# gereonsuch/gr-FDC

Measured on AMD Instinct MI355X. Metric: complex Msamples/s in, 64k-FFT/256-ch overlap-save; achieved HBM GB/s vs peak, higher is better.
Workload: dtype f32

## Files before the change

### gr-fdc_amd/csrc/fdc_block256.hip

```cpp
#include "fdc_blockcommon.hpp"
#include "fdc_iq.hpp"

namespace fdc {

extern __shared__ __attribute__((aligned(16))) unsigned char fdc_smem_blk[];

typedef unsigned long long u8v __attribute__((ext_vector_type(8)));

template <int P>
struct BlkGeom {
    static_assert(P == 2 || P == 4 || P == 8, "passes of 32 columns: N = 16384, 32768 or 65536");
    static constexpr int kN1 = 32 * P;
    static constexpr int kN = 256 * kN1;
    static constexpr int kJT = P == 8 ? 4 : 8;
    static constexpr int kJB = P == 8 ? 2 : P == 4 ? 4 : 8;
    static constexpr int kLd = P == 2 ? 32 * P + 2 : 32 * P + 6;
    static constexpr int kTripBytes = 16 * kJT * kLd * 8;
    static constexpr int kOffCt = kTripBytes > kStripsEnd ? kTripBytes : kStripsEnd;
    static constexpr int kOffWrow = P == 8 ? 136960 : kOffCt + 32 * P * 8;
    static constexpr int kOffB = kOffWrow + 16 * 18 * 8;
    static constexpr int kOffSA = kOffB + 32 * 18 * 8;
    static constexpr int kOffSoff = kOffSA + 16 * P * 18 * 8;
    static constexpr int kLds = kOffSoff + kN1 * 4;
    static constexpr int kOffSoffOff = kOffSA + 16 * P * 16 * 8;
    static constexpr int kOffWrowF = kOffSoffOff + kN1 * 4;
    static constexpr int kLdsOff = kOffWrowF + 16 * 18 * 8;
    static_assert(kLdsOff <= 160 * 1024 && kLds <= 160 * 1024, "LDS budget");
    static_assert(kOffCt >= kStripsEnd && kOffCt + 32 * P * 8 <= kOffWrow, "stage-2 trip buffer and twiddles below the tables, tables above the strips");
    static_assert((16 * (kJB - 1) * kLd + 32 * (P - 1)) * 8 < 65536, "ds offsets of a base register");
};


template <int P, bool NT, bool OFF, bool FWD, bool R4 = false, bool HALF = false, class TI = float2, class TO = float2>
__global__ FDC_PLAIN_DS __launch_bounds__(512, (P == 2 && !OFF && !R4 && !FWD) ? 4 : 2) void k_blk256(const TI *__restrict__ in, size_t in_stride, TO *__restrict__ out,
                                                const float2 *__restrict__ tw256, const float2 *__restrict__ twq,
                                                const float2 *__restrict__ cbt, const float *__restrict__ shn,
                                                const long long *__restrict__ slot_off, long long out_base,
                                                long long nb_call, unsigned out_bytes, int nb, int hints,
                                                unsigned long long *__restrict__ dbg , int roff, long long first_block,
                                                float2 *__restrict__ fwd_scratch, const unsigned *__restrict__ keep,
                                                typename IqTail<TI, TO>::type gpow )
{
    typedef BlkGeom<P> GM;
    constexpr bool kIq = !std::is_same<TI, float2>::value, kOq = !std::is_same<TO, float2>::value;
    static_assert(!kIq || !FWD, "integer input: the channelizer forms (the forward transform takes widened input)");
    static_assert(!kOq || !FWD, "integer output: the channelizer forms");
    constexpr unsigned kEs = (unsigned)sizeof(TI);
    constexpr unsigned kOs = (unsigned)sizeof(TO);
    [[maybe_unused]] const float iq_scale = iq_tail_scale(gpow);
    [[maybe_unused]] const float oq_scale = oq_tail_scale(gpow);
    static_assert(!HALF || (!OFF && !FWD), "the half-slot form is a variant of the on-grid channelizer");
    constexpr int kN1 = GM::kN1, kLd = GM::kLd, kJT = GM::kJT, kJB = GM::kJB;
    float2 *scr = reinterpret_cast<float2 *>(fdc_smem_blk);
    float2 *wrow = reinterpret_cast<float2 *>(fdc_smem_blk + GM::kOffWrow);
    float2 *Bt = reinterpret_cast<float2 *>(fdc_smem_blk + GM::kOffB);
    float2 *SA = reinterpret_cast<float2 *>(fdc_smem_blk + GM::kOffSA);
    constexpr int kSaLd = OFF ? 16 : 18;
    unsigned *soff = reinterpret_cast<unsigned *>(fdc_smem_blk + (OFF ? GM::kOffSoffOff : GM::kOffSoff));
    float2 *ctab = reinterpret_cast<float2 *>(fdc_smem_blk + GM::kOffCt);
    const int tid = threadIdx.x;
    const int w = tid >> 6, lane = tid & 63, col = lane & 3, b = lane >> 2, c5 = 4 * w + col;
    unsigned mqs[4] = {~0u, ~0u, ~0u, ~0u};
    if (FWD && keep) {
        const int wu = __builtin_amdgcn_readfirstlane(w) % P;
#pragma unroll
        for (int q = 0; q < 4; q++) mqs[q] = keep[wu * 4 + q];
    }

    const int grid = gridDim.x, first = xcd_first_block();
    if (first >= nb) return;

    constexpr unsigned inbytes = (unsigned)GM::kN * kEs;
    constexpr unsigned kRowGrp = (unsigned)kN1 * 16u * kEs;
    const unsigned voff = (unsigned)(b * kN1 + c5) * kEs;
    [[maybe_unused]] auto ld_in = [&](__amdgpu_buffer_rsrc_t r, unsigned soff, auto aux) __attribute__((always_inline)) -> cf {
        constexpr int kAux = decltype(aux)::value;
        if constexpr (sizeof(TI) == 4) return mk(__uint_as_float(__builtin_amdgcn_raw_buffer_load_b32(r, voff, soff, kAux)), 0.f);
        else return mk(__uint_as_float((unsigned)__builtin_amdgcn_raw_buffer_load_b16(r, voff, soff, kAux)), 0.f);
    };
    const __amdgpu_buffer_rsrc_t rcb = make_rsrc(cbt, (unsigned)kN1 * 16u * 8u);
    const unsigned voffc = (unsigned)(c5 * 16 + b) * 8u;
    cf LA[16], LB[16], cbA, cbB;
    {
        const __amdgpu_buffer_rsrc_t rin = make_rsrc(in + (size_t)first * in_stride, inbytes);
#pragma unroll
        for (int a = 0; a < 16; a++) {
            if constexpr (kIq) LA[a] = ld_in(rin, (unsigned)a * kRowGrp, std::integral_constant<int, 0>{});
            else LA[a] = bld2(rin, voff, (unsigned)a * kRowGrp);
        }
        cbA = bld2(rcb, voffc, 0);
    }
    float2 *wrowF = OFF ? reinterpret_cast<float2 *>(fdc_smem_blk + GM::kOffWrowF) : wrow;
    const int r16 = roff & 15;
    for (int i = tid; i < 256; i += 512) {
        wrow[(i >> 4) * 18 + (i & 15)] = tw256[((i >> 4) * (i & 15)) & 255];
        if (OFF)
            wrowF[(i >> 4) * 18 + (i & 15)] = tw256[((i >> 4) * ((((i & 15) - r16) & 15) + roff)) & 255];
    }
    for (int i = tid; i < kN1; i += 512) {
        const long long o = slot_off[i];
        soff[(i % P) * 32 + ((i / P) & 1) * 16 + rev16((i / P) >> 1)] = o >= 0 ? (unsigned)((o * nb_call + out_base) * kOs) : 0xFFFFFFFFu;
    }
    for (int i = tid; i < 32 * P; i += 512) ctab[i] = tw256[((i / P) * (i % P) * (8 / P)) & 255];
    Bt[(tid >> 4) * 18 + (tid & 15)] = twq[HALF ? tid ^ 8 : tid];
    for (int i = tid; i < 256 * P; i += 512) {
        const int ps = i >> 8, bb = (i >> 4) & 15, q = i & 15, qt = HALF ? q ^ 8 : q;
        const float2 t = twq[(size_t)(32 * ps) * 16 + qt];
        const float s = shn[bb + 16 * qt];
        SA[(ps * 16 + bb) * kSaLd + q] = make_float2(t.x * s, t.y * s);
    }
    __syncthreads();

    float2 *const scrw = scr + w * kStripPts + lane;
    const float2 *const scrr = scr + w * kStripPts + col + 68 * b;
    const float2 *const wr = wrow + b * 18;
    const float2 *const wrf = wrowF + b * 18;
    const float2 *const btr = Bt + c5 * 18;
    const __amdgpu_buffer_rsrc_t rout = make_rsrc(out, out_bytes);
    constexpr bool kScr = FWD || R4;
    const __amdgpu_buffer_rsrc_t rscr = make_rsrc(kScr ? fwd_scratch + (size_t)blockIdx.x * 32768 : fwd_scratch, kScr ? 32768u * 8u : 0u);


    for (int m = first; m < nb; m += grid) {
        const int mnext = m + grid < nb ? m + grid : m;
        const float sgn = (OFF && !R4 && (roff & 1) && ((first_block + m) & 1)) ? -1.0f : 1.0f;
        cf phs = mk(1.f, 0.f);
        if constexpr (OFF && R4) {
            const int pc = (int)((((first_block + m) & 3) * (roff & 3)) & 3);
            phs = mk(pc == 0 ? 1.f : pc == 2 ? -1.f : 0.f, pc == 1 ? 1.f : pc == 3 ? -1.f : 0.f);
        }
        typedef unsigned long long gvec __attribute__((ext_vector_type(P)));
        gvec G[8];
#define FDC_GGET(j, ps) unpack_cf(G[j][ps])
#define FDC_GPUT(j, ps, val) G[j][ps] = pack_cf(val)
        auto one_pass = [&](const int ps, cf (&cur)[16], const cf cbc, cf (&L)[16], cf &cbn) __attribute__((always_inline)) {
            const cf cb = (OFF && R4) ? cmul(cbc, phs) : OFF ? cbc * sgn : cbc;
            const int pn = ps < P - 1 ? ps + 1 : 0;
            const int mb = ps < P - 1 ? m : mnext;
            const __amdgpu_buffer_rsrc_t rin = make_rsrc(in + (size_t)mb * in_stride + 32 * pn, inbytes);
            if constexpr (kIq) {
                if (hints & 2) {
#pragma unroll
                    for (int a = 0; a < 16; a++) L[a] = ld_in(rin, (unsigned)a * kRowGrp, std::integral_constant<int, 2>{});
                } else {
#pragma unroll
                    for (int a = 0; a < 16; a++) L[a] = ld_in(rin, (unsigned)a * kRowGrp, std::integral_constant<int, 0>{});
                }
            } else if (hints & 2) {
#pragma unroll
                for (int a = 0; a < 16; a++) L[a] = bld2_nt(rin, voff, (unsigned)a * kRowGrp);
            } else {
#pragma unroll
                for (int a = 0; a < 16; a++) L[a] = bld2(rin, voff, (unsigned)a * kRowGrp);
            }
            cbn = bld2(rcb, voffc, (unsigned)pn * 4096u);
            if constexpr (kIq) {
#pragma unroll
                for (int a = 0; a < 16; a++) cur[a] = iq_widen_bits(TI{}, __float_as_uint(cur[a].x), iq_scale);
            }
            dft16<false>(cur);
            cf tw[16];
#pragma unroll
            for (int i = 0; i < 8; i++) {
                const float4 t = ld4(&wrf[2 * i]);
                tw[2 * i] = mk(t.x, t.y); tw[2 * i + 1] = mk(t.z, t.w);
            }
            if (OFF) {
#pragma unroll
                for (int p = 0; p < 16; p++) st2(&scrw[68 * ((p - r16) & 15)], cmul(cur[rev16(p)], tw[p]));
            } else {
                st2(&scrw[0], cur[rev16(0)]);
#pragma unroll
                for (int p = 1; p < 16; p++) st2(&scrw[68 * p], cmul(cur[rev16(p)], tw[p]));
            }
            __builtin_amdgcn_wave_barrier();
            cf v[16];
            strip_get(v, scrr);
            if constexpr (FWD) {
                dft16<false>(v);
                const float2 *sar = SA + (ps * 16 + b) * kSaLd;
#pragma unroll
                for (int i = 0; i < 8; i++) {
                    const float4 t0 = ld4(&btr[2 * i]), t1 = ld4(&sar[2 * i]);
                    const cf y0 = cmul(cmul(cmul(v[rev16(2 * i)], mk(t0.x, t0.y)), mk(t1.x, t1.y)), cb);
                    const cf y1 = cmul(cmul(cmul(v[rev16(2 * i + 1)], mk(t0.z, t0.w)), mk(t1.z, t1.w)), cb);
                    if (i < 4) { FDC_GPUT(2 * i, ps, y0); FDC_GPUT(2 * i + 1, ps, y1); }
                    else {
                        bst2(rscr, (unsigned)tid * 8u + (unsigned)(2 * i - 8) * 4096u, (unsigned)ps * 32768u, y0);
                        bst2(rscr, (unsigned)tid * 8u + (unsigned)(2 * i - 7) * 4096u, (unsigned)ps * 32768u, y1);
                    }
                }
            } else {
                dft16<false>(v);
                cf u[16];
                {
                    const float2 *sar = SA + (ps * 16 + b) * kSaLd;
#pragma unroll
                    for (int i = 0; i < 8; i++) {
                        const float4 t0 = ld4(&btr[2 * i]), t1 = ld4(&sar[2 * i]);
                        u[HALF ? 2 * i : (2 * i) ^ 8] = cmul(cmul(v[rev16(2 * i)], mk(t0.x, t0.y)), mk(t1.x, t1.y));
                        u[HALF ? 2 * i + 1 : (2 * i + 1) ^ 8] = cmul(cmul(v[rev16(2 * i + 1)], mk(t0.z, t0.w)), mk(t1.z, t1.w));
                    }
                }
                dft16<true>(u);
#pragma unroll
                for (int i = 0; i < 8; i++) {
                    const float4 t = ld4(&wr[2 * i]);
                    tw[2 * i] = mk(t.x, t.y); tw[2 * i + 1] = mk(t.z, t.w);
                }
                u[rev16(0)] = cmul(u[rev16(0)], cb);
#pragma unroll
                for (int p = 1; p < 16; p++) u[rev16(p)] = cmul(cmulc(u[rev16(p)], tw[p]), cb);
                strip_trip(u, scrw, scrr);
                dft16<true>(u);
#pragma unroll
                for (int j = 0; j < 8; j++) FDC_GPUT(j, ps, u[rev16(8 + j)]);
                if constexpr (R4) {
#pragma unroll
                    for (int j = 0; j < 4; j++) bst2(rscr, (unsigned)tid * 8u + (unsigned)j * 4096u, (unsigned)ps * 16384u, u[rev16(4 + j)]);
                }
            }
        };
        if constexpr (OFF && P == 8) {
#pragma nounroll
            for (int ps = 0; ps < P; ps++) {
                cf cur[16];
#pragma unroll
                for (int a = 0; a < 16; a++) cur[a] = LA[a];
                one_pass(ps, cur, cbA, LA, cbA);
            }
        } else {
#pragma nounroll
            for (int pp = 0; pp < P; pp += 2) {
                one_pass(pp, LA, cbA, LB, cbB);
                one_pass(pp + 1, LB, cbB, LA, cbA);
            }
        }
        auto stage2 = [&](auto get, const int rowbase, auto njc) __attribute__((always_inline)) {
            constexpr int kNJ = decltype(njc)::value;
            constexpr int kNTrip = (kNJ + kJT - 1) / kJT;
            __syncthreads();
            int t2 = tid;
            asm volatile("" : "+v"(t2));
            const int lane2 = t2 & 63, w2 = __builtin_amdgcn_readfirstlane(t2 >> 6), b_2 = lane2 >> 2, c5_2 = 4 * w2 + (lane2 & 3);
            const int klo2 = w2 % P, rh2 = w2 / P;
            float2 *const gw0 = scr + b_2 * kLd + c5_2;
            int rowjb = 16 * kJB * kLd;
            asm volatile("" : "+v"(rowjb));
            float2 *const gw1 = gw0 + rowjb;
            const float2 *const gr = scr + (64 * rh2 + lane2) * kLd + 32 * klo2;
            const uint4 *const sow = reinterpret_cast<const uint4 *>(soff + 32 * klo2);
#pragma unroll
            for (int tr = 0; tr < kNTrip; tr++) {
                const int ja = kNJ - kJT * tr < kJT ? kNJ - kJT * tr : kJT;
                cf ct[P];
                {
                    const float2 *ctr = reinterpret_cast<const float2 *>(fdc_smem_blk + GM::kOffCt) + c5_2 * P;
#pragma unroll
                    for (int i = 0; i < P / 2; i++) {
                        const float4 t = ld4(&ctr[2 * i]);
                        ct[2 * i] = mk(t.x, t.y); ct[2 * i + 1] = mk(t.z, t.w);
                    }
                }
                cf src[kJT][P];
#pragma unroll
                for (int jj = 0; jj < kJT; jj++)
#pragma unroll
                    for (int ps = 0; ps < P; ps++) if (jj < ja) src[jj][ps] = get(kJT * tr + jj, ps);
#pragma unroll
                for (int jj = 0; jj < kJT; jj++) {
                    if (jj >= ja) continue;
                    cf a[P];
#pragma unroll
                    for (int ps = 0; ps < P; ps++) a[ps] = src[jj][ps];
                    pass_dft<P>(a);
                    float2 *const gw = (jj < kJB ? gw0 : gw1) + (jj % kJB) * 16 * kLd;
                    st2(&gw[0], a[0]);
#pragma unroll
                    for (int k = 1; k < P; k++) st2(&gw[32 * k], cmul(a[pass_idx<P>(k)], ct[k]));
                }
                __builtin_amdgcn_sched_barrier(0);
                __syncthreads();
                const bool reads = P == 8 || 4 * rh2 < ja;
                cf v[32];
                if (reads) {
#pragma unroll
                    for (int i = 0; i < 16; i++) {
                        const float4 t = ld4(&gr[2 * i]);
                        v[2 * i] = mk(t.x, t.y); v[2 * i + 1] = mk(t.z, t.w);
                    }
                }
                __syncthreads();
                __builtin_amdgcn_sched_barrier(0);
                if (reads) {
                    dft32<false>(v);
                    const int trow0 = 16 * kJT * tr + 64 * rh2, trow = trow0 + lane2;
                    const unsigned rb = (unsigned)(m * (FWD ? GM::kN : (R4 ? 192 : 128)) + rowbase + trow) * kOs;
                    unsigned mq = FWD ? mqs[((rowbase + trow0) >> 6) & 3] : ~0u;
                    if constexpr (FWD) asm volatile("" : "+s"(mq));
#pragma unroll
                    for (int q = 0; q < 8; q++) {
                        const uint4 t = sow[q];
                        const unsigned so[4] = {t.x, t.y, t.z, t.w};
#pragma unroll
                        for (int e = 0; e < 4; e++) {
                            const unsigned o = FWD ? (so[e] | (((mq >> (4 * q + e)) & 1u) - 1u)) : so[e];
                            if constexpr (kOq) {
                                const unsigned u = oq_bits(TO{}, v[4 * q + e], oq_scale);
                                if constexpr (kOs == 4) __builtin_amdgcn_raw_buffer_store_b32(u, rout, (o == 0xFFFFFFFFu ? 0xFFFFFFF0u : o + rb), 0, NT ? 2 : 0);
                                else __builtin_amdgcn_raw_buffer_store_b16((unsigned short)u, rout, (o == 0xFFFFFFFFu ? 0xFFFFFFF0u : o + rb), 0, NT ? 2 : 0);
                            } else
                                bst2t<NT>(rout, (o == 0xFFFFFFFFu ? 0xFFFFFFF0u : o + rb), v[4 * q + e]);
                        }
                    }
                    if constexpr (FWD) {
                        if (gpow) {
                            float t16[16];
#pragma unroll
                            for (int i = 0; i < 16; i++) {
                                const float s0 = __builtin_fmaf(v[i].y, v[i].y, v[i].x * v[i].x);
                                const float s1 = __builtin_fmaf(v[i + 16].y, v[i + 16].y, v[i + 16].x * v[i + 16].x);
                                asm("s_nop 1\n\tv_add_f32_dpp %0, %1, %1 row_ror:8 row_mask:0xf bank_mask:0x3\n\t"
                                    "v_add_f32_dpp %0, %2, %2 row_ror:8 row_mask:0xf bank_mask:0xc" : "=&v"(t16[i]) : "v"(s0), "v"(s1));
                            }
                            float t8[8];
#pragma unroll
                            for (int i = 0; i < 8; i++)
                                asm("s_nop 1\n\tv_add_f32_dpp %0, %1, %1 row_shl:4 row_mask:0xf bank_mask:0x5\n\t"
                                    "v_add_f32_dpp %0, %2, %2 row_shr:4 row_mask:0xf bank_mask:0xa" : "=&v"(t8[i]) : "v"(t16[i]), "v"(t16[i + 8]));
                            const bool b1 = (lane2 & 2) != 0, b0 = (lane2 & 1) != 0;
                            float t4[4], t2[2];
#pragma unroll
                            for (int i = 0; i < 4; i++) {
                                const float keepv = b1 ? t8[i + 4] : t8[i], send = b1 ? t8[i] : t8[i + 4];
                                t4[i] = keepv + __builtin_bit_cast(float, __builtin_amdgcn_update_dpp(0, __builtin_bit_cast(int, send), 0x4E , 0xF, 0xF, false));
                            }
#pragma unroll
                            for (int i = 0; i < 2; i++) {
                                const float keepv = b0 ? t4[i + 2] : t4[i], send = b0 ? t4[i] : t4[i + 2];
                                t2[i] = keepv + __builtin_bit_cast(float, __builtin_amdgcn_update_dpp(0, __builtin_bit_cast(int, send), 0xB1 , 0xF, 0xF, false));
                            }
                            const int i16 = lane2 & 15, rho = lane2 >> 4, gsrc = 2 * (i16 & 1);
                            const int a0 = (16 * gsrc + 4 * rho + (i16 >> 2)) * 4, a1 = a0 + 64;
                            const int z0 = __builtin_bit_cast(int, t2[0]), z1 = __builtin_bit_cast(int, t2[1]);
                            const int f0a = __builtin_amdgcn_ds_bpermute(a0, z0), f0b = __builtin_amdgcn_ds_bpermute(a0, z1);
                            const int f1a = __builtin_amdgcn_ds_bpermute(a1, z0), f1b = __builtin_amdgcn_ds_bpermute(a1, z1);
                            const bool odd = (i16 & 2) != 0;
                            float2 pr;
                            pr.x = __builtin_bit_cast(float, odd ? f0b : f0a);
                            pr.y = __builtin_bit_cast(float, odd ? f1b : f1a);
                            const int reg = 8 * rho + (i16 >> 1), slot = klo2 + P * ((reg >> 4) + 2 * (4 * (reg & 3) + ((reg & 15) >> 2)));
                            *reinterpret_cast<float2 *>(gpow + (size_t)m * (GM::kN / 16) + 16 * slot + (rowbase + trow0) / 16 + gsrc) = pr;
                        }
                    }
                }
                __builtin_amdgcn_sched_barrier(0);
            }
        };
        stage2([&](int j, int ps) { return FDC_GGET(j, ps); }, R4 ? 64 : 0, std::integral_constant<int, 8>{});
        if constexpr (FWD) {
            asm volatile("s_waitcnt vmcnt(0)" ::: "memory");
            stage2([&](int j, int ps) { return bld2_sc1(rscr, (unsigned)tid * 8u + (unsigned)(j * 4096 + ps * 32768), 0u); }, 128,
                   std::integral_constant<int, 8>{});
        }
        if constexpr (R4) {
            asm volatile("s_waitcnt vmcnt(0)" ::: "memory");
            stage2([&](int j, int ps) { return bld2_sc1(rscr, (unsigned)tid * 8u + (unsigned)(j * 4096 + ps * 16384), 0u); }, 0,
                   std::integral_constant<int, 4>{});
        }
    }
}

template <class TI>
static hipError_t init_block_kernels_in()
{
    hipError_t e;
#define FDC_SETB(P, A, B, R4) \
    e = hipFuncSetAttribute(reinterpret_cast<const void *>(k_blk256<P, A, B, false, R4, false, TI>), hipFuncAttributeMaxDynamicSharedMemorySize, \
                            B ? BlkGeom<P>::kLdsOff : BlkGeom<P>::kLds); \
    if (e != hipSuccess) return e;
#define FDC_SETH(P, A, R4) \
    e = hipFuncSetAttribute(reinterpret_cast<const void *>(k_blk256<P, A, false, false, R4, true, TI>), hipFuncAttributeMaxDynamicSharedMemorySize, BlkGeom<P>::kLds); \
    if (e != hipSuccess) return e;
#define FDC_SETP(P) \
    FDC_SETB(P, true, false, false) FDC_SETB(P, false, false, false) FDC_SETB(P, true, true, false) FDC_SETB(P, false, true, false) \
    FDC_SETB(P, true, false, true) FDC_SETB(P, false, false, true) FDC_SETB(P, true, true, true) FDC_SETB(P, false, true, true) \
    FDC_SETH(P, true, false) FDC_SETH(P, false, false) FDC_SETH(P, true, true) FDC_SETH(P, false, true)
    FDC_SETP(2) FDC_SETP(4) FDC_SETP(8)
#undef FDC_SETP
#undef FDC_SETH
#undef FDC_SETB
    return hipSuccess;
}

template <class TI, class TO> struct kOqR4Narrowed {
    static constexpr bool value = std::is_same<TI, float2>::value && !std::is_same<TO, float2>::value;
};

template <class TI, class TO>
static hipError_t init_block_kernels_oq()
{
    hipError_t e;
#define FDC_SETB(P, B, R4) \
    e = hipFuncSetAttribute(reinterpret_cast<const void *>(k_blk256<P, true, B, false, R4, false, TI, TO>), hipFuncAttributeMaxDynamicSharedMemorySize, \
                            B ? BlkGeom<P>::kLdsOff : BlkGeom<P>::kLds); \
    if (e != hipSuccess) return e;
#define FDC_SETH(P, R4) \
    e = hipFuncSetAttribute(reinterpret_cast<const void *>(k_blk256<P, true, false, false, R4, true, TI, TO>), hipFuncAttributeMaxDynamicSharedMemorySize, BlkGeom<P>::kLds); \
    if (e != hipSuccess) return e;
#define FDC_SETP(P) \
    FDC_SETB(P, false, false) FDC_SETB(P, true, false) FDC_SETB(P, false, true) FDC_SETB(P, true, true) FDC_SETH(P, false) FDC_SETH(P, true)
    FDC_SETP(2) FDC_SETP(4)
    FDC_SETB(8, false, false) FDC_SETB(8, true, false) FDC_SETH(8, false)
    if constexpr (!kOqR4Narrowed<TI, TO>::value) { FDC_SETB(8, false, true) FDC_SETB(8, true, true) FDC_SETH(8, true) }
#undef FDC_SETP
#undef FDC_SETH
#undef FDC_SETB
    return hipSuccess;
}

hipError_t init_block_kernels()
{
    hipError_t e = init_block_kernels_in<sc16>();
    if (e != hipSuccess) return e;
    if ((e = init_block_kernels_in<sc8>()) != hipSuccess) return e;
    if ((e = init_block_kernels_oq<float2, sc16>()) != hipSuccess) return e;
    if ((e = init_block_kernels_oq<float2, sc8>()) != hipSuccess) return e;
    if ((e = init_block_kernels_oq<sc16, sc16>()) != hipSuccess) return e;
    if ((e = init_block_kernels_oq<sc16, sc8>()) != hipSuccess) return e;
    if ((e = init_block_kernels_oq<sc8, sc16>()) != hipSuccess) return e;
    if ((e = init_block_kernels_oq<sc8, sc8>()) != hipSuccess) return e;
#define FDC_SETB(P, A, B, F, R4) \
    e = hipFuncSetAttribute(reinterpret_cast<const void *>(k_blk256<P, A, B, F, R4>), hipFuncAttributeMaxDynamicSharedMemorySize, \
                            B ? BlkGeom<P>::kLdsOff : BlkGeom<P>::kLds); \
    if (e != hipSuccess) return e;
#define FDC_SETP(P) \
    FDC_SETB(P, true, false, false, false) FDC_SETB(P, false, false, false, false) FDC_SETB(P, true, true, false, false) \
    FDC_SETB(P, false, true, false, false) FDC_SETB(P, true, false, false, true) FDC_SETB(P, false, false, false, true) \
    FDC_SETB(P, true, true, false, true) FDC_SETB(P, false, true, false, true)
    FDC_SETP(2) FDC_SETP(4) FDC_SETP(8)
    FDC_SETB(8, true, false, true, false) FDC_SETB(8, false, false, true, false) FDC_SETB(4, true, false, true, false) FDC_SETB(4, false, false, true, false)
    FDC_SETB(2, true, false, true, false) FDC_SETB(2, false, false, true, false)
#undef FDC_SETP
#undef FDC_SETB
#define FDC_SETH(P, A, R4) \
    e = hipFuncSetAttribute(reinterpret_cast<const void *>(k_blk256<P, A, false, false, R4, true>), hipFuncAttributeMaxDynamicSharedMemorySize, BlkGeom<P>::kLds); \
    if (e != hipSuccess) return e;
#define FDC_SETHP(P) FDC_SETH(P, true, false) FDC_SETH(P, false, false) FDC_SETH(P, true, true) FDC_SETH(P, false, true)
    FDC_SETHP(2) FDC_SETHP(4) FDC_SETHP(8)
#undef FDC_SETHP
#undef FDC_SETH
    return hipSuccess;
}

bool poly_block_supports(int N) { return N == 16384 || N == 32768 || N == 65536; }

template <class TI, class TO = float2>
static hipError_t poly_block_in(const BlockLaunch &b, const TI *in, TO *out, float iq_scale, float oq_scale = 1.0f)
{
    if (b.nb_chunk <= 0) return hipSuccess;
    if (b.L != 256 || b.r < 0 || b.r >= 256) return hipErrorInvalidValue;
    constexpr bool kIq = !std::is_same<TI, float2>::value, kOq = !std::is_same<TO, float2>::value;
    const bool nt = (b.hints & 1) != 0, r4 = b.R == 4;
    if (kOq && !nt) return hipErrorInvalidValue;
    auto iq_tail = [](float si, float so) -> typename IqTail<TI, TO>::type {
        if constexpr (!kIq && !kOq) return (void)si, (void)so, (float *)nullptr;
        else if constexpr (kIq && kOq) return make_float2(si, so);
        else if constexpr (kIq) return (void)so, si;
        else return (void)si, so;
    };
    const bool halfslot = b.half();
    if (!poly_block_supports(b.N) || (b.R != 2 && !r4) || (r4 && !b.scratch)) return hipErrorInvalidValue;
    const int grid = b.grid(b.N == 16384 && b.R == 2 && (!b.r || halfslot) ? 2 : 1);
#define FDC_L(P, A, O, R4, H, roff) \
    hipExtLaunchKernelGGL((k_blk256<P, A || kOq, O, false, R4, H, TI, TO>), dim3((unsigned)grid), dim3(512), O ? BlkGeom<P>::kLdsOff : BlkGeom<P>::kLds, b.s, \
                          b.ev_start, b.ev_stop, 0u, in, b.in_stride, out, b.tw256, b.twq, b.cbt, b.shn, b.slot_off, (long long)b.mbase * (R4 ? 192 : 128), \
                          (long long)b.nb_call, b.out_bytes, b.nb_chunk, b.hints, (unsigned long long *)nullptr, roff, b.first_block, \
                          R4 ? b.scratch : (float2 *)nullptr, (const unsigned *)nullptr, iq_tail(iq_scale, oq_scale))
#define FDC_LB(P, A, O, R4) FDC_L(P, A, O, R4, false, b.r)
#define FDC_LH(P, A, R4) FDC_L(P, A, false, R4, true, 0)
#define FDC_R4(P) if constexpr (P != 8 || !kOqR4Narrowed<TI, TO>::value)
#define FDC_LP(P) \
    do { \
        if (halfslot) { \
            if (r4) { FDC_R4(P) { if (nt) FDC_LH(P, true, true); else FDC_LH(P, false, true); } else return hipErrorInvalidValue; } \
            else { if (nt) FDC_LH(P, true, false); else FDC_LH(P, false, false); } \
        } else if (r4 && b.r) { FDC_R4(P) { if (nt) FDC_LB(P, true, true, true); else FDC_LB(P, false, true, true); } else return hipErrorInvalidValue; } \
        else if (r4) { FDC_R4(P) { if (nt) FDC_LB(P, true, false, true); else FDC_LB(P, false, false, true); } else return hipErrorInvalidValue; } \
        else if (b.r) { if (nt) FDC_LB(P, true, true, false); else FDC_LB(P, false, true, false); } \
        else { if (nt) FDC_LB(P, true, false, false); else FDC_LB(P, false, false, false); } \
    } while (0)
    if (b.N == 65536) FDC_LP(8); else if (b.N == 32768) FDC_LP(4); else FDC_LP(2);
#undef FDC_LP
#undef FDC_R4
#undef FDC_LH
#undef FDC_LB
#undef FDC_L
    return hipGetLastError();
}

hipError_t launch_poly_block(const BlockLaunch &b) { return poly_block_in(b, b.in, b.out, 1.0f); }

hipError_t launch_poly_block_iq(const BlockLaunch &b, int fmt, float scale, const void *in)
{
    if (fmt == kIqSc16) return poly_block_in(b, static_cast<const sc16 *>(in), b.out, scale);
    if (fmt == kIqSc8) return poly_block_in(b, static_cast<const sc8 *>(in), b.out, scale);
    return hipErrorInvalidValue;
}

template <class TO>
static hipError_t poly_block_oq_in(const BlockLaunch &b, int ifmt, float iscale, const void *in, TO *out, float oscale)
{
    if (ifmt == kIqFloat) return poly_block_in<float2, TO>(b, static_cast<const float2 *>(in), out, 1.0f, oscale);
    if (ifmt == kIqSc16) return poly_block_in<sc16, TO>(b, static_cast<const sc16 *>(in), out, iscale, oscale);
    if (ifmt == kIqSc8) return poly_block_in<sc8, TO>(b, static_cast<const sc8 *>(in), out, iscale, oscale);
    return hipErrorInvalidValue;
}

hipError_t launch_poly_block_oq(const BlockLaunch &b, int ifmt, float iscale, const void *in, int ofmt, float oscale, void *out)
{
    if (ofmt == kIqSc16) return poly_block_oq_in(b, ifmt, iscale, in, static_cast<sc16 *>(out), oscale);
    if (ofmt == kIqSc8) return poly_block_oq_in(b, ifmt, iscale, in, static_cast<sc8 *>(out), oscale);
    return hipErrorInvalidValue;
}

hipError_t launch_block_fft(int N, const float2 *in, size_t in_stride, float2 *out, int nitems, const float2 *tw256,
                            const float2 *twq, const float2 *cbt0, const float *shn1, const long long *slot_off,
                            float2 *scratch , int ncu, int hints, hipStream_t s, hipEvent_t *ev,
                            const unsigned *keep, float *gpow )
{
    if (!poly_block_supports(N)) return hipErrorInvalidValue;
    const int per = (int)(((size_t)1 << 28) / (size_t)N);
    for (int m0 = 0; m0 < nitems; m0 += per) {
        const int nb = nitems - m0 < per ? nitems - m0 : per;
        int grid = ncu > 0 ? ncu : 256;
        if (grid > nb) grid = nb;
        hipEvent_t e0 = ev && m0 == 0 ? ev[0] : nullptr, e2 = ev && m0 + nb >= nitems ? ev[1] : nullptr;
#define FDC_LF(P, A) \
        hipExtLaunchKernelGGL((k_blk256<P, A, false, true>), dim3((unsigned)grid), dim3(512), BlkGeom<P>::kLds, s, e0, e2, 0u, in + (size_t)m0 * in_stride, \
                              in_stride, out + (size_t)m0 * (size_t)N, tw256, twq, cbt0, shn1, slot_off, 0ll, 1ll, \
                              (unsigned)((size_t)nb * (size_t)N * 8), nb, hints, (unsigned long long *)nullptr, 0, 0ll, scratch, keep, \
                              gpow ? gpow + (size_t)m0 * (size_t)(N / 16) : (float *)nullptr)
        const bool nt = (hints & 1) != 0;
        if (N == 65536) { if (nt) FDC_LF(8, true); else FDC_LF(8, false); }
        else if (N == 32768) { if (nt) FDC_LF(4, true); else FDC_LF(4, false); }
        else { if (nt) FDC_LF(2, true); else FDC_LF(2, false); }
#undef FDC_LF
    }
    if (ev) { hipError_t e = hipEventRecord(ev[2], s); if (e != hipSuccess) return e; }
    return hipGetLastError();
}

}
```

### gr-fdc_amd/csrc/fdc_blockcommon.hpp

```cpp
#pragma once
#include <hip/hip_ext.h>
#include <type_traits>
#include "fdc_kernels.h"
#include "fdc_radix16.hpp"
#include "fdc_devutil.hpp"

namespace fdc {

__device__ __forceinline__ unsigned long long pack_cf(cf v) { return ((unsigned long long)__float_as_uint(v.y) << 32) | __float_as_uint(v.x); }
__device__ __forceinline__ cf unpack_cf(unsigned long long u) { return mk(__uint_as_float((unsigned)u), __uint_as_float((unsigned)(u >> 32))); }
#if defined(__HIP_DEVICE_COMPILE__)
#define FDC_PLAIN_DS __attribute__((target("no-load-store-opt")))
#else
#define FDC_PLAIN_DS
#endif

__device__ __forceinline__ cf quad_xor1(cf x)
{
    return mk(__int_as_float(__builtin_amdgcn_update_dpp(0, __float_as_int(x.x), 0xB1, 0xF, 0xF, true)),
              __int_as_float(__builtin_amdgcn_update_dpp(0, __float_as_int(x.y), 0xB1, 0xF, 0xF, true)));
}
__device__ __forceinline__ cf quad_xor2(cf x)
{
    return mk(__int_as_float(__builtin_amdgcn_update_dpp(0, __float_as_int(x.x), 0x4E, 0xF, 0xF, true)),
              __int_as_float(__builtin_amdgcn_update_dpp(0, __float_as_int(x.y), 0x4E, 0xF, 0xF, true)));
}

template <int P> __device__ __forceinline__ constexpr int pass_idx(int k) { return P == 8 ? 4 * (k & 1) + (k >> 1) : k; }
template <int P>
__device__ __forceinline__ void pass_dft(cf (&a)[P])
{
    if constexpr (P == 8) dft8<false>(a);
    else if constexpr (P == 4) dft4<false>(a[0], a[1], a[2], a[3]);
    else { const cf s0 = a[0] + a[1], d0 = a[0] - a[1]; a[0] = s0; a[1] = d0; }
}

__device__ __forceinline__ int xcd_first_block()
{
    const int grid = gridDim.x, per = grid >> 3;
    const bool xmap = (grid & 7) == 0;
    return xmap ? (int)(blockIdx.x & 7) * per + (int)(blockIdx.x >> 3) : (int)blockIdx.x;
}

template <int n>
__device__ __forceinline__ void ld_row(cf (&t)[n], const float2 *row)
{
#pragma unroll
    for (int i = 0; i < n / 2; i++) {
        const float4 q = ld4(&row[2 * i]);
        t[2 * i] = mk(q.x, q.y); t[2 * i + 1] = mk(q.z, q.w);
    }
}

constexpr int kStripPts = 1084;
constexpr int kStripsEnd = 8 * kStripPts * 8;
__device__ __forceinline__ void strip_get(cf (&v)[16], const float2 *scrr)
{
#pragma unroll
    for (int bb = 0; bb < 16; bb++) v[bb] = ld2(&scrr[4 * bb]);
}
__device__ __forceinline__ void strip_trip(cf (&u)[16], float2 *scrw, const float2 *scrr)
{
    __builtin_amdgcn_wave_barrier();
#pragma unroll
    for (int p = 0; p < 16; p++) st2(&scrw[68 * p], u[rev16(p)]);
    __builtin_amdgcn_wave_barrier();
    strip_get(u, scrr);
}
__device__ __forceinline__ void strip_fft256(cf (&cur)[16], cf (&v)[16], const float2 *wr, float2 *scrw, const float2 *scrr)
{
    dft16<false>(cur);
    {
        cf tw[16];
        ld_row(tw, wr);
        st2(&scrw[0], cur[rev16(0)]);
#pragma unroll
        for (int p = 1; p < 16; p++) st2(&scrw[68 * p], cmul(cur[rev16(p)], tw[p]));
    }
    __builtin_amdgcn_wave_barrier();
    strip_get(v, scrr);
    dft16<false>(v);
}
__device__ __forceinline__ void strip_ifft256(cf (&u)[16], const float2 *wr, float2 *scrw, const float2 *scrr)
{
    dft16<true>(u);
    {
        cf tw[16];
        ld_row(tw, wr);
#pragma unroll
        for (int p = 1; p < 16; p++) u[rev16(p)] = cmulc(u[rev16(p)], tw[p]);
    }
    strip_trip(u, scrw, scrr);
    dft16<true>(u);
}
constexpr int kEvery = -1;
template <int... Vs, class F>
inline void for_values(int v, F &&f)
{
    ((v == kEvery || v == Vs ? f(std::integral_constant<int, Vs>{}) : void()), ...);
}
template <class F>
inline void for_block_variants(int nt, int r4, int p, F &&f)
{
    for_values<8, 4, 2>(p, [&](auto P) {
        for_values<0, 1>(r4, [&](auto R4) { for_values<1, 0>(nt, [&](auto NT) { f(NT, R4, P); }); });
    });
}
inline hipError_t set_block_lds(const void *kernel, int bytes)
{
    return hipFuncSetAttribute(kernel, hipFuncAttributeMaxDynamicSharedMemorySize, bytes);
}

}
```

Baseline: 202,100.

## Factor stage-2 twiddle/window tables into small LDS tables and drop per-pass cbt loads

```diff
diff --git a/gr-fdc_amd/csrc/fdc_block256.hip b/gr-fdc_amd/csrc/fdc_block256.hip
--- a/gr-fdc_amd/csrc/fdc_block256.hip
+++ b/gr-fdc_amd/csrc/fdc_block256.hip
@@ -18,12 +18,14 @@
     static constexpr int kTripBytes = 16 * kJT * kLd * 8;
     static constexpr int kOffCt = kTripBytes > kStripsEnd ? kTripBytes : kStripsEnd;
     static constexpr int kOffWrow = P == 8 ? 136960 : kOffCt + 32 * P * 8;
-    static constexpr int kOffB = kOffWrow + 16 * 18 * 8;
-    static constexpr int kOffSA = kOffB + 32 * 18 * 8;
-    static constexpr int kOffSoff = kOffSA + 16 * P * 18 * 8;
-    static constexpr int kLds = kOffSoff + kN1 * 4;
-    static constexpr int kOffSoffOff = kOffSA + 16 * P * 16 * 8;
-    static constexpr int kOffWrowF = kOffSoffOff + kN1 * 4;
+    static constexpr bool kSplit = P > 2;
+    static constexpr int kOffLT = kOffWrow + 16 * 18 * 8;
+    static constexpr int kOffUR = kOffLT + 64 * 18 * 8;
+    static constexpr int kOffB = kOffLT, kOffSA = kOffB + 32 * 18 * 8;
+    static constexpr int kOffSoff = kSplit ? kOffUR + kN1 * 4 * 8 : kOffSA + 16 * P * 18 * 8;
+    static constexpr int kOffCbl = kOffSoff + kN1 * 4;
+    static constexpr int kLds = kOffCbl + (kSplit ? (P + 8) * 16 * 8 : 0);
+    static constexpr int kOffWrowF = kLds;
     static constexpr int kLdsOff = kOffWrowF + 16 * 18 * 8;
     static_assert(kLdsOff <= 160 * 1024 && kLds <= 160 * 1024, "LDS budget");
     static_assert(kOffCt >= kStripsEnd && kOffCt + 32 * P * 8 <= kOffWrow, "stage-2 trip buffer and twiddles below the tables, tables above the strips");
@@ -53,10 +55,13 @@
     constexpr int kN1 = GM::kN1, kLd = GM::kLd, kJT = GM::kJT, kJB = GM::kJB;
     float2 *scr = reinterpret_cast<float2 *>(fdc_smem_blk);
     float2 *wrow = reinterpret_cast<float2 *>(fdc_smem_blk + GM::kOffWrow);
+    constexpr bool kSplit = GM::kSplit;
+    float2 *LT = reinterpret_cast<float2 *>(fdc_smem_blk + GM::kOffLT);
+    float2 *UR = reinterpret_cast<float2 *>(fdc_smem_blk + GM::kOffUR);
+    float2 *CBL = reinterpret_cast<float2 *>(fdc_smem_blk + GM::kOffCbl);
     float2 *Bt = reinterpret_cast<float2 *>(fdc_smem_blk + GM::kOffB);
     float2 *SA = reinterpret_cast<float2 *>(fdc_smem_blk + GM::kOffSA);
-    constexpr int kSaLd = OFF ? 16 : 18;
-    unsigned *soff = reinterpret_cast<unsigned *>(fdc_smem_blk + (OFF ? GM::kOffSoffOff : GM::kOffSoff));
+    unsigned *soff = reinterpret_cast<unsigned *>(fdc_smem_blk + GM::kOffSoff);
     float2 *ctab = reinterpret_cast<float2 *>(fdc_smem_blk + GM::kOffCt);
     const int tid = threadIdx.x;
     const int w = tid >> 6, lane = tid & 63, col = lane & 3, b = lane >> 2, c5 = 4 * w + col;
@@ -78,9 +83,9 @@
         if constexpr (sizeof(TI) == 4) return mk(__uint_as_float(__builtin_amdgcn_raw_buffer_load_b32(r, voff, soff, kAux)), 0.f);
         else return mk(__uint_as_float((unsigned)__builtin_amdgcn_raw_buffer_load_b16(r, voff, soff, kAux)), 0.f);
     };
-    const __amdgpu_buffer_rsrc_t rcb = make_rsrc(cbt, (unsigned)kN1 * 16u * 8u);
-    const unsigned voffc = (unsigned)(c5 * 16 + b) * 8u;
-    cf LA[16], LB[16], cbA, cbB;
+    [[maybe_unused]] const __amdgpu_buffer_rsrc_t rcb = make_rsrc(cbt, (unsigned)kN1 * 16u * 8u);
+    [[maybe_unused]] const unsigned voffc = (unsigned)(c5 * 16 + b) * 8u;
+    cf LA[16], LB[16], cbA = mk(1.f, 0.f), cbB = cbA;
     {
         const __amdgpu_buffer_rsrc_t rin = make_rsrc(in + (size_t)first * in_stride, inbytes);
 #pragma unroll
@@ -88,26 +93,40 @@
             if constexpr (kIq) LA[a] = ld_in(rin, (unsigned)a * kRowGrp, std::integral_constant<int, 0>{});
             else LA[a] = bld2(rin, voff, (unsigned)a * kRowGrp);
         }
-        cbA = bld2(rcb, voffc, 0);
+        if constexpr (!kSplit) cbA = bld2(rcb, voffc, 0);
     }
     float2 *wrowF = OFF ? reinterpret_cast<float2 *>(fdc_smem_blk + GM::kOffWrowF) : wrow;
     const int r16 = roff & 15;
     for (int i = tid; i < 256; i += 512) {
-        wrow[(i >> 4) * 18 + (i & 15)] = tw256[((i >> 4) * (i & 15)) & 255];
+        const int ip = (i >> 4) * 18 + (((i & 15) - 1) & 15);
+        wrow[ip] = tw256[((i >> 4) * (i & 15)) & 255];
         if (OFF)
-            wrowF[(i >> 4) * 18 + (i & 15)] = tw256[((i >> 4) * ((((i & 15) - r16) & 15) + roff)) & 255];
+            wrowF[ip] = tw256[((i >> 4) * ((((i & 15) - r16) & 15) + roff)) & 255];
     }
     for (int i = tid; i < kN1; i += 512) {
         const long long o = slot_off[i];
         soff[(i % P) * 32 + ((i / P) & 1) * 16 + rev16((i / P) >> 1)] = o >= 0 ? (unsigned)((o * nb_call + out_base) * kOs) : 0xFFFFFFFFu;
     }
     for (int i = tid; i < 32 * P; i += 512) ctab[i] = tw256[((i / P) * (i % P) * (8 / P)) & 255];
-    Bt[(tid >> 4) * 18 + (tid & 15)] = twq[HALF ? tid ^ 8 : tid];
-    for (int i = tid; i < 256 * P; i += 512) {
-        const int ps = i >> 8, bb = (i >> 4) & 15, q = i & 15, qt = HALF ? q ^ 8 : q;
-        const float2 t = twq[(size_t)(32 * ps) * 16 + qt];
-        const float s = shn[bb + 16 * qt];
-        SA[(ps * 16 + bb) * kSaLd + q] = make_float2(t.x * s, t.y * s);
+    if constexpr (kSplit) {
+        for (int i = tid; i < 1024; i += 512) {
+            const int ln = i >> 4, q = i & 15, qt = HALF ? q ^ 8 : q;
+            const float2 t = twq[(ln & 3) * 16 + qt];
+            const float s = shn[(ln >> 2) + 16 * qt];
+            const float2 e = make_float2(t.x * s, t.y * s), c = cbt[(ln & 3) * 16 + (ln >> 2)];
+            LT[ln * 18 + q] = make_float2(e.x * c.x - e.y * c.y, e.x * c.y + e.y * c.x);
+        }
+        for (int i = tid; i < kN1 * 4; i += 512) UR[i] = twq[(i >> 4) * 64 + (HALF ? (i & 15) ^ 8 : i & 15)];
+        if (tid < (P + 8) * 16)
+            CBL[tid] = cbt[(tid < P * 16 ? (tid >> 4) * 512 : ((tid >> 4) - P) * 64) + (tid & 15)];
+    } else {
+        Bt[(tid >> 4) * 18 + (tid & 15)] = twq[HALF ? tid ^ 8 : tid];
+        for (int i = tid; i < 256 * P; i += 512) {
+            const int ps = i >> 8, bb = (i >> 4) & 15, q = i & 15, qt = HALF ? q ^ 8 : q;
+            const float2 t = twq[(size_t)(32 * ps) * 16 + qt];
+            const float s = shn[bb + 16 * qt];
+            SA[(ps * 16 + bb) * 18 + q] = make_float2(t.x * s, t.y * s);
+        }
     }
     __syncthreads();
 
@@ -115,7 +134,9 @@
     const float2 *const scrr = scr + w * kStripPts + col + 68 * b;
     const float2 *const wr = wrow + b * 18;
     const float2 *const wrf = wrowF + b * 18;
-    const float2 *const btr = Bt + c5 * 18;
+    const float2 *const tr0 = kSplit ? UR + w * 16 : Bt + c5 * 18;
+    const float2 *const tr1 = kSplit ? LT + lane * 18 : SA + b * 18;
+    const float2 *const cblr = CBL + b;
     const __amdgpu_buffer_rsrc_t rout = make_rsrc(out, out_bytes);
     constexpr bool kScr = FWD || R4;
     const __amdgpu_buffer_rsrc_t rscr = make_rsrc(kScr ? fwd_scratch + (size_t)blockIdx.x * 32768 : fwd_scratch, kScr ? 32768u * 8u : 0u);
@@ -134,7 +155,8 @@
 #define FDC_GGET(j, ps) unpack_cf(G[j][ps])
 #define FDC_GPUT(j, ps, val) G[j][ps] = pack_cf(val)
         auto one_pass = [&](const int ps, cf (&cur)[16], const cf cbc, cf (&L)[16], cf &cbn) __attribute__((always_inline)) {
-            const cf cb = (OFF && R4) ? cmul(cbc, phs) : OFF ? cbc * sgn : cbc;
+            const cf cbl = kSplit ? cmul(ld2(&cblr[16 * ps]), ld2(&cblr[16 * (P + w)])) : cbc;
+            const cf cb = (OFF && R4) ? cmul(cbl, phs) : OFF ? cbl * sgn : cbl;
             const int pn = ps < P - 1 ? ps + 1 : 0;
             const int mb = ps < P - 1 ? m : mnext;
             const __amdgpu_buffer_rsrc_t rin = make_rsrc(in + (size_t)mb * in_stride + 32 * pn, inbytes);
@@ -153,19 +175,16 @@
 #pragma unroll
                 for (int a = 0; a < 16; a++) L[a] = bld2(rin, voff, (unsigned)a * kRowGrp);
             }
-            cbn = bld2(rcb, voffc, (unsigned)pn * 4096u);
+            if constexpr (!kSplit) cbn = bld2(rcb, voffc, (unsigned)pn * 4096u);
+            const float2 *const r0 = tr0 + (kSplit ? 128 * ps : 0), *const r1 = tr1 + (kSplit ? 0 : 288 * ps);
             if constexpr (kIq) {
 #pragma unroll
                 for (int a = 0; a < 16; a++) cur[a] = iq_widen_bits(TI{}, __float_as_uint(cur[a].x), iq_scale);
             }
             dft16<false>(cur);
             cf tw[16];
-#pragma unroll
-            for (int i = 0; i < 8; i++) {
-                const float4 t = ld4(&wrf[2 * i]);
-                tw[2 * i] = mk(t.x, t.y); tw[2 * i + 1] = mk(t.z, t.w);
-            }
-            if (OFF) {
+            ld_row_sh<OFF>(tw, wrf);
+            if constexpr (OFF) {
 #pragma unroll
                 for (int p = 0; p < 16; p++) st2(&scrw[68 * ((p - r16) & 15)], cmul(cur[rev16(p)], tw[p]));
             } else {
@@ -178,10 +197,9 @@
             strip_get(v, scrr);
             if constexpr (FWD) {
                 dft16<false>(v);
-                const float2 *sar = SA + (ps * 16 + b) * kSaLd;
 #pragma unroll
                 for (int i = 0; i < 8; i++) {
-                    const float4 t0 = ld4(&btr[2 * i]), t1 = ld4(&sar[2 * i]);
+                    const float4 t0 = ld4(&r0[2 * i]), t1 = ld4(&r1[2 * i]);
                     const cf y0 = cmul(cmul(cmul(v[rev16(2 * i)], mk(t0.x, t0.y)), mk(t1.x, t1.y)), cb);
                     const cf y1 = cmul(cmul(cmul(v[rev16(2 * i + 1)], mk(t0.z, t0.w)), mk(t1.z, t1.w)), cb);
                     if (i < 4) { FDC_GPUT(2 * i, ps, y0); FDC_GPUT(2 * i + 1, ps, y1); }
@@ -194,20 +212,15 @@
                 dft16<false>(v);
                 cf u[16];
                 {
-                    const float2 *sar = SA + (ps * 16 + b) * kSaLd;
 #pragma unroll
                     for (int i = 0; i < 8; i++) {
-                        const float4 t0 = ld4(&btr[2 * i]), t1 = ld4(&sar[2 * i]);
+                        const float4 t0 = ld4(&r0[2 * i]), t1 = ld4(&r1[2 * i]);
                         u[HALF ? 2 * i : (2 * i) ^ 8] = cmul(cmul(v[rev16(2 * i)], mk(t0.x, t0.y)), mk(t1.x, t1.y));
                         u[HALF ? 2 * i + 1 : (2 * i + 1) ^ 8] = cmul(cmul(v[rev16(2 * i + 1)], mk(t0.z, t0.w)), mk(t1.z, t1.w));
                     }
                 }
                 dft16<true>(u);
-#pragma unroll
-                for (int i = 0; i < 8; i++) {
-                    const float4 t = ld4(&wr[2 * i]);
-                    tw[2 * i] = mk(t.x, t.y); tw[2 * i + 1] = mk(t.z, t.w);
-                }
+                ld_row_sh<false>(tw, wr);
                 u[rev16(0)] = cmul(u[rev16(0)], cb);
 #pragma unroll
                 for (int p = 1; p < 16; p++) u[rev16(p)] = cmul(cmulc(u[rev16(p)], tw[p]), cb);
diff --git a/gr-fdc_amd/csrc/fdc_blockcommon.hpp b/gr-fdc_amd/csrc/fdc_blockcommon.hpp
--- a/gr-fdc_amd/csrc/fdc_blockcommon.hpp
+++ b/gr-fdc_amd/csrc/fdc_blockcommon.hpp
@@ -50,6 +50,21 @@
         const float4 q = ld4(&row[2 * i]);
         t[2 * i] = mk(q.x, q.y); t[2 * i + 1] = mk(q.z, q.w);
     }
+}
+
+template <bool WRAP>
+__device__ __forceinline__ void ld_row_sh(cf (&t)[16], const float2 *row)
+{
+#pragma unroll
+    for (int i = 0; i < 7; i++) {
+        const float4 q = ld4(&row[2 * i]);
+        t[2 * i + 1] = mk(q.x, q.y); t[2 * i + 2] = mk(q.z, q.w);
+    }
+    if constexpr (WRAP) {
+        const float4 q = ld4(&row[14]);
+        t[15] = mk(q.x, q.y); t[0] = mk(q.z, q.w);
+    } else
+        t[15] = ld2(&row[14]);
 }
 
 constexpr int kStripPts = 1084;
```

Measured after the change: 210,400 (median of 6 runs). +4.1%, better.
